# alipay/PainlessInferenceAcceleration

Hardware: NVIDIA H100
Metric: accepted tokens/sec @ Llama-2-7B 64-draft/8-branch; mean accepted len/step (higher is better)
Workload: dtype bf16

## Files before the change

painlessinferenceacceleration_b200/csrc/fused_ops.cu:

```cuda
#include <cuda_bf16.h>

#include "common.cuh"

namespace pia {
namespace fused {

__device__ __forceinline__ float bf(float x) { return __bfloat162float(__float2bfloat16_rn(x)); }

union Pack8 { uint4 u; __nv_bfloat16 h[8]; };

__device__ __forceinline__ Pack8 load_x8(const __nv_bfloat16 *x, const float *parts, int n_parts, long long part_stride,
                                         long long off) {
  Pack8 a;
  if (parts == nullptr) { a.u = *reinterpret_cast<const uint4 *>(x + off); return a; }
  float acc[8] = {0.f, 0.f, 0.f, 0.f, 0.f, 0.f, 0.f, 0.f};
  for (int s = 0; s < n_parts; ++s) {
    const float4 lo = *reinterpret_cast<const float4 *>(parts + s * part_stride + off);
    const float4 hi = *reinterpret_cast<const float4 *>(parts + s * part_stride + off + 4);
    acc[0] += lo.x; acc[1] += lo.y; acc[2] += lo.z; acc[3] += lo.w;
    acc[4] += hi.x; acc[5] += hi.y; acc[6] += hi.z; acc[7] += hi.w;
  }
#pragma unroll
  for (int j = 0; j < 8; ++j) a.h[j] = __float2bfloat16_rn(acc[j]);
  return a;
// ... 41 lines not shown
#pragma unroll
  for (int i = 0; i < 16; ++i) tot += red[i];
  const float inv = rsqrtf(tot / (float)hidden + eps);
  const uint4 *wv = reinterpret_cast<const uint4 *>(w);
  uint4 *yv = reinterpret_cast<uint4 *>(y + row_off);
#pragma unroll
  for (int k = 0; k < kRmsVec; ++k) {
    const int v = tid + k * 512;
    if (v < nvec) {
      Pack8 ww; ww.u = wv[v];
      Pack8 o;
#pragma unroll
      for (int j = 0; j < 8; ++j) {
        const float xh = __bfloat162float(keep[k].h[j]) * inv;
        o.h[j] = __float2bfloat16_rn(__bfloat162float(ww.h[j]) * (kRoundTwice ? bf(xh) : xh));
      }
      yv[v] = o.u;
    }
  }
}

enum { ROPE_HALF = 0, ROPE_INTERLEAVED = 1, ROPE_HALF_F32 = 2, ROPE_NONE = 3 };

__device__ __forceinline__ int tree_pos(const unsigned long long *mask, int mask_words, int i, int P, int pad_len,
                                        int max_pos) {
  int depth = -1;
  for (int w = 0; w < mask_words; ++w) depth += __popcll(mask[(long long)i * mask_words + w]);
  int pos = (P > pad_len ? P - pad_len : 0) + depth;
  if (pos < 0) pos = 0;
  if (pos >= max_pos) pos = max_pos - 1;
  return pos;
}

template <int kLayout, bool kLogn = false>
__global__ void __launch_bounds__(256) k_rope_kv_append(const __nv_bfloat16 *qkv, const unsigned long long *mask,
                                                        int mask_words, pia_slots_t sl,
                                                        int hq, int hkv, int hd, const void *cos_t,
                                                        const void *sin_t, int max_pos, __nv_bfloat16 *q_out,
                                                        __nv_bfloat16 *kc, __nv_bfloat16 *vc, int max_seq,
                                                        int rotary_dim, const __nv_bfloat16 *q_scale, int hd_src,
                                                        float q_mul) {
  static_assert(!kLogn || kLayout == ROPE_HALF_F32, "log-n scaling is built on the fp32 layout only");
  pdl_launch_dependents();
  pdl_wait();
  const int i = blockIdx.x;
  const int slot = i / sl.rows_per_slot, node = i % sl.rows_per_slot;
  const int n = sl.d_n[slot], P = sl.d_prefix_len[slot];
  const int pad_len = sl.d_pad_len ? sl.d_pad_len[slot] : 0;
  if (node >= n) return;
  kc += (long long)slot * sl.kv_slot_stride;
  vc += (long long)slot * sl.kv_slot_stride;
  if constexpr (kLayout == ROPE_NONE) {
    const int cpr = hd >> 3, cache_row = P + node;
    const __nv_bfloat16 *src = qkv + (long long)i * (hq + 2 * hkv) * hd_src;
    for (int c = threadIdx.x; c < (hq + 2 * hkv) * cpr; c += blockDim.x) {
      const int head = c / cpr, d0 = (c % cpr) * 8;
      Pack8 a;
      a.u = d0 < hd_src ? *reinterpret_cast<const uint4 *>(src + head * hd_src + d0) : make_uint4(0, 0, 0, 0);
      if (head < hq) {
#pragma unroll
        for (int j = 0; j < 8; ++j) a.h[j] = __float2bfloat16_rn(__fmul_rn(__bfloat162float(a.h[j]), q_mul));
        *reinterpret_cast<uint4 *>(q_out + ((long long)i * hq + head) * hd + d0) = a.u;
      } else if (head < hq + hkv) {
        *reinterpret_cast<uint4 *>(kc + ((long long)(head - hq) * max_seq + cache_row) * hd + d0) = a.u;
      } else {
        *reinterpret_cast<uint4 *>(vc + ((long long)(head - hq - hkv) * max_seq + cache_row) * hd + d0) = a.u;
      }
    }
    return;
  }
  const int pos = tree_pos(mask, mask_words, i, P, pad_len, max_pos);
  const int half = hd >> 1, cpr = hd >> 3;
  const int row_elems = (hq + 2 * hkv) * hd;
  const __nv_bfloat16 *src = qkv + (long long)i * row_elems;
  const int cache_row = P + node;
  const int total = (hq + 2 * hkv) * cpr;
  for (int c = threadIdx.x; c < total; c += blockDim.x) {
    const int head = c / cpr, ch = c % cpr;
    const int d0 = ch * 8;
    Pack8 a; a.u = *reinterpret_cast<const uint4 *>(src + head * hd + d0);
    if (head < hq + hkv) {
      Pack8 o;
      const __nv_bfloat16 *cos_b = static_cast<const __nv_bfloat16 *>(cos_t);
      const __nv_bfloat16 *sin_b = static_cast<const __nv_bfloat16 *>(sin_t);
      if constexpr (kLayout == ROPE_INTERLEAVED) {
        o = a;
        if (d0 < rotary_dim) {
          const int rhalf = rotary_dim >> 1;
          union { uint2 u; __nv_bfloat16 h[4]; } cs, sn;
          cs.u = *reinterpret_cast<const uint2 *>(cos_b + (long long)pos * rhalf + (d0 >> 1));
          sn.u = *reinterpret_cast<const uint2 *>(sin_b + (long long)pos * rhalf + (d0 >> 1));
#pragma unroll
          for (int j = 0; j < 4; ++j) {
            const float x0 = __bfloat162float(a.h[2 * j]), x1 = __bfloat162float(a.h[2 * j + 1]);
            const float c = __bfloat162float(cs.h[j]), s = __bfloat162float(sn.h[j]);
            o.h[2 * j] = __float2bfloat16_rn(bf(x0 * c) + bf(-x1 * s));
            o.h[2 * j + 1] = __float2bfloat16_rn(bf(x1 * c) + bf(x0 * s));
          }
        }
      } else if constexpr (kLayout == ROPE_HALF_F32) {
        const int dp = d0 < half ? d0 + half : d0 - half;
        Pack8 b; b.u = *reinterpret_cast<const uint4 *>(src + head * hd + dp);
        const float *cf = static_cast<const float *>(cos_t) + (long long)pos * half + d0 % half;
        const float *sf = static_cast<const float *>(sin_t) + (long long)pos * half + d0 % half;
        float c[8], s[8];
        *reinterpret_cast<float4 *>(c) = *reinterpret_cast<const float4 *>(cf);
        *reinterpret_cast<float4 *>(c + 4) = *reinterpret_cast<const float4 *>(cf + 4);
        *reinterpret_cast<float4 *>(s) = *reinterpret_cast<const float4 *>(sf);
        *reinterpret_cast<float4 *>(s + 4) = *reinterpret_cast<const float4 *>(sf + 4);
#pragma unroll
// ... 195 lines not shown
                              (const __nv_bfloat16 *)d_weight, eps, hidden, (__nv_bfloat16 *)d_residual_out,
                              (__nv_bfloat16 *)d_y));
  count_launch();
  return PIA_OK;
}

extern "C" int pia_rmsnorm(const void *d_x, const void *d_residual_in, const void *d_weight, float eps, int rounding,
                           int rows, int hidden, void *d_residual_out, void *d_y, void *stream) {
  PIA_REQUIRE(d_x, "bad rmsnorm arguments");
  return rmsnorm(d_x, nullptr, 0, 0ll, d_residual_in, d_weight, eps, rounding, rows, hidden, d_residual_out, d_y,
                 stream);
}

extern "C" int pia_rmsnorm_partials(const float *d_x_parts, int n_parts, int64_t part_stride, const void *d_residual_in,
                                    const void *d_weight, float eps, int rounding, int rows, int hidden,
                                    void *d_residual_out, void *d_y, void *stream) {
  PIA_REQUIRE(d_x_parts && n_parts >= 1, "bad rmsnorm arguments");
  return rmsnorm(nullptr, d_x_parts, n_parts, (long long)part_stride, d_residual_in, d_weight, eps, rounding, rows,
                 hidden, d_residual_out, d_y, stream);
}

template <int kLayout, bool kLogn = false>
static int rope_kv_append(const void *d_qkv, const uint64_t *d_mask, int mask_words, const pia_slots_t *slots,
                          int n_q_heads, int n_kv_heads, int head_dim, const void *d_cos, const void *d_sin, int max_pos,
                          void *d_q_out, void *d_k_cache_layer, void *d_v_cache_layer, int max_seq, int rotary_dim,
                          void *stream, const void *d_q_scale = nullptr, int hd_src = 0, float q_mul = 1.f) {
  PIA_REQUIRE(d_qkv && d_mask && slots && slots->d_n && slots->d_prefix_len && d_q_out && d_k_cache_layer &&
                  d_v_cache_layer && (kLayout == ROPE_NONE || (d_cos && d_sin)), "null argument");
  PIA_REQUIRE(slots->batch >= 1 && slots->rows_per_slot >= 1 && slots->kv_slot_stride >= 0, "bad slot table");
  PIA_REQUIRE(head_dim % 16 == 0 && mask_words >= 1 && mask_words <= 2, "bad rope arguments");
  PIA_REQUIRE(!kLogn || d_q_scale, "null argument");
  PIA_REQUIRE(kLayout != ROPE_NONE || (hd_src >= 8 && hd_src % 8 == 0 && hd_src <= head_dim),
              "bad source head width: a positive multiple of 8, at most head_dim");
  PIA_CUDA_CHECK(launch_kernel(k_rope_kv_append<kLayout, kLogn>, dim3(slots->batch * slots->rows_per_slot), dim3(256), 0,
                              (cudaStream_t)stream, (const __nv_bfloat16 *)d_qkv, (const unsigned long long *)d_mask,
                              mask_words, *slots, n_q_heads, n_kv_heads, head_dim, d_cos, d_sin, max_pos,
                              (__nv_bfloat16 *)d_q_out,
                              (__nv_bfloat16 *)d_k_cache_layer, (__nv_bfloat16 *)d_v_cache_layer, max_seq, rotary_dim,
                              (const __nv_bfloat16 *)d_q_scale, hd_src, q_mul));
  count_launch();
  return PIA_OK;
}

extern "C" int pia_kv_append_qscale(const void *d_qkv, const uint64_t *d_mask, int mask_words, const pia_slots_t *slots,
                                    int n_q_heads, int n_kv_heads, int src_head_dim, int head_dim, float q_mul,
                                    void *d_q_out, void *d_k_cache_layer, void *d_v_cache_layer, int max_seq,
                                    void *stream) {
  return rope_kv_append<ROPE_NONE>(d_qkv, d_mask, mask_words, slots, n_q_heads, n_kv_heads, head_dim, nullptr, nullptr,
                                   1, d_q_out, d_k_cache_layer, d_v_cache_layer, max_seq, head_dim, stream, nullptr,
                                   src_head_dim, q_mul);
}

extern "C" int pia_learned_pos_embed(const void *d_tok_table, const int32_t *d_ids, const void *d_pos_table,
                                     int offset, int max_pos, const uint64_t *d_mask, int mask_words,
                                     const pia_slots_t *slots, int hidden, void *d_out, void *stream) {
  PIA_REQUIRE(d_pos_table && d_mask && slots && slots->d_n && slots->d_prefix_len && d_out &&
                  (d_ids || !d_tok_table), "null argument");
  PIA_REQUIRE(slots->batch >= 1 && slots->rows_per_slot >= 1, "bad slot table");
  PIA_REQUIRE(hidden > 0 && hidden % 8 == 0 && offset >= 0 && max_pos >= 1 && mask_words >= 1 && mask_words <= 2,
              "bad position embedding arguments: hidden a positive multiple of 8, offset >= 0, max_pos >= 1");
  PIA_CUDA_CHECK(launch_kernel(k_learned_pos_embed, dim3(slots->batch * slots->rows_per_slot), dim3(256), 0,
                              (cudaStream_t)stream, (const __nv_bfloat16 *)d_tok_table, (const int *)d_ids,
                              (const __nv_bfloat16 *)d_pos_table, offset, max_pos, (const unsigned long long *)d_mask,
                              mask_words, *slots, hidden, (__nv_bfloat16 *)d_out));
  count_launch();
  return PIA_OK;
}
// ... 209 lines not shown
```

painlessinferenceacceleration_b200/csrc/tree_attn.cu:

```cuda
#include <cuda.h>
#include <cuda_bf16.h>

#include <stdlib.h>

#include <new>

#include "common.cuh"

namespace pia {
namespace attn {

constexpr int BN = 128;
constexpr int NSTAGE = 2;
constexpr int NTHREADS = 288;
constexpr int PRODUCER_WARP = 8;
constexpr int SUB = 128 * 128;
constexpr int MAX_SPLIT = 8;
constexpr int ALIBI_SLOPE = 64;
constexpr int ALIBI_DEPTH = 128;
constexpr float LOG2E = 1.4426950408889634f;

template <int HD>
struct Smem {
  static constexpr int TILE_BYTES = HD / 64 * SUB;
  static constexpr int Q = 0, K = TILE_BYTES, V = K + NSTAGE * TILE_BYTES;
  static constexpr int BAR = V + NSTAGE * TILE_BYTES;
  static constexpr int MRG_ACC = 0;
  static constexpr int MRG_ML = 7 * TILE_BYTES / 2;
  static constexpr int DED_ACC = BAR + 256, DED_ACC_BYTES = (64 + MAX_SPLIT) * HD * 4,
                       DED_ML = DED_ACC + DED_ACC_BYTES;
  static constexpr int TOTAL = DED_ML + 1024 + 1024;
  static_assert(MRG_ACC + HD / 4 * (128 + MAX_SPLIT) * 16 <= MRG_ML, "aliased partial rows overlap the (m, l) pairs");
  static_assert(MRG_ML + (128 + MAX_SPLIT) * 8 <= BAR, "aliased merge area reaches the barriers");
  static_assert(3 * NSTAGE * 8 <= ALIBI_SLOPE && ALIBI_SLOPE + 8 <= ALIBI_DEPTH && BAR + ALIBI_DEPTH + 128 <= DED_ACC,
                "ALiBi slopes / depths overlap");
};

__device__ __forceinline__ uint32_t smem_u32(const void *p) { return (uint32_t)__cvta_generic_to_shared(p); }
__device__ __forceinline__ void mbar_init(uint32_t bar, int count) {
  asm volatile("mbarrier.init.shared::cta.b64 [%0], %1;" ::"r"(bar), "r"(count));
}
__device__ __forceinline__ void mbar_arrive(uint32_t bar) {
  asm volatile("mbarrier.arrive.shared::cta.b64 _, [%0];" ::"r"(bar) : "memory");
}
__device__ __forceinline__ void mbar_expect_tx(uint32_t bar, uint32_t bytes) {
  asm volatile("mbarrier.arrive.expect_tx.shared::cta.b64 _, [%0], %1;" ::"r"(bar), "r"(bytes) : "memory");
}
__device__ __forceinline__ void mbar_wait(uint32_t bar, uint32_t parity) {
  uint32_t done;
  do {
    asm volatile(
        "{\n\t.reg .pred p;\n\t"
        "mbarrier.try_wait.parity.shared::cta.b64 p, [%1], %2;\n\t"
        "selp.u32 %0, 1, 0, p;\n\t}"
        : "=r"(done)
        : "r"(bar), "r"(parity)
        : "memory");
  } while (!done);
}
__device__ __forceinline__ void tma_load_3d(uint32_t dst, const CUtensorMap *map, uint32_t bar, int c0, int c1, int c2) {
  asm volatile(
      "cp.async.bulk.tensor.3d.shared::cluster.global.mbarrier::complete_tx::bytes [%0], [%1, {%3, %4, %5}], [%2];"
      ::"r"(dst), "l"(map), "r"(bar), "r"(c0), "r"(c1), "r"(c2)
      : "memory");
}
__device__ __forceinline__ void wgmma_fence() { asm volatile("wgmma.fence.sync.aligned;" ::: "memory"); }
__device__ __forceinline__ void wgmma_commit() { asm volatile("wgmma.commit_group.sync.aligned;" ::: "memory"); }
__device__ __forceinline__ void wgmma_wait_all() { asm volatile("wgmma.wait_group.sync.aligned 0;" ::: "memory"); }
// ... 20 lines not shown
      "{\n\t"
      "wgmma.mma_async.sync.aligned.m64n128k16.f32.bf16.bf16 "
      "{%0, %1, %2, %3, %4, %5, %6, %7, %8, %9, %10, %11, %12, %13, %14, %15, %16, %17, %18, %19, %20, %21, %22, %23, %24, %25, %26, %27, %28, %29, %30, %31, %32, %33, %34, %35, %36, %37, %38, %39, %40, %41, %42, %43, %44, %45, %46, %47, %48, %49, %50, %51, %52, %53, %54, %55, %56, %57, %58, %59, %60, %61, %62, %63}, {%64, %65, %66, %67}, %68, 1, 1, 1, 1;\n\t}"
      : "+f"(d[0]), "+f"(d[1]), "+f"(d[2]), "+f"(d[3]), "+f"(d[4]), "+f"(d[5]), "+f"(d[6]), "+f"(d[7]), "+f"(d[8]), "+f"(d[9]), "+f"(d[10]), "+f"(d[11]), "+f"(d[12]), "+f"(d[13]), "+f"(d[14]), "+f"(d[15]), "+f"(d[16]), "+f"(d[17]), "+f"(d[18]), "+f"(d[19]), "+f"(d[20]), "+f"(d[21]), "+f"(d[22]), "+f"(d[23]), "+f"(d[24]), "+f"(d[25]), "+f"(d[26]), "+f"(d[27]), "+f"(d[28]), "+f"(d[29]), "+f"(d[30]), "+f"(d[31]), "+f"(d[32]), "+f"(d[33]), "+f"(d[34]), "+f"(d[35]), "+f"(d[36]), "+f"(d[37]), "+f"(d[38]), "+f"(d[39]), "+f"(d[40]), "+f"(d[41]), "+f"(d[42]), "+f"(d[43]), "+f"(d[44]), "+f"(d[45]), "+f"(d[46]), "+f"(d[47]), "+f"(d[48]), "+f"(d[49]), "+f"(d[50]), "+f"(d[51]), "+f"(d[52]), "+f"(d[53]), "+f"(d[54]), "+f"(d[55]), "+f"(d[56]), "+f"(d[57]), "+f"(d[58]), "+f"(d[59]), "+f"(d[60]), "+f"(d[61]), "+f"(d[62]), "+f"(d[63])
      : "r"(a[0]), "r"(a[1]), "r"(a[2]), "r"(a[3]), "l"(desc_b)
      : "memory");
}
__device__ __forceinline__ void wgmma_pv(float (&d)[32], const uint32_t *a, uint64_t desc_b) {
  asm volatile(
      "{\n\t"
      "wgmma.mma_async.sync.aligned.m64n64k16.f32.bf16.bf16 "
      "{%0, %1, %2, %3, %4, %5, %6, %7, %8, %9, %10, %11, %12, %13, %14, %15, %16, %17, %18, %19, %20, %21, %22, %23, %24, %25, %26, %27, %28, %29, %30, %31}, {%32, %33, %34, %35}, %36, 1, 1, 1, 1;\n\t}"
      : "+f"(d[0]), "+f"(d[1]), "+f"(d[2]), "+f"(d[3]), "+f"(d[4]), "+f"(d[5]), "+f"(d[6]), "+f"(d[7]), "+f"(d[8]), "+f"(d[9]), "+f"(d[10]), "+f"(d[11]), "+f"(d[12]), "+f"(d[13]), "+f"(d[14]), "+f"(d[15]), "+f"(d[16]), "+f"(d[17]), "+f"(d[18]), "+f"(d[19]), "+f"(d[20]), "+f"(d[21]), "+f"(d[22]), "+f"(d[23]), "+f"(d[24]), "+f"(d[25]), "+f"(d[26]), "+f"(d[27]), "+f"(d[28]), "+f"(d[29]), "+f"(d[30]), "+f"(d[31])
      : "r"(a[0]), "r"(a[1]), "r"(a[2]), "r"(a[3]), "l"(desc_b)
      : "memory");
}
__device__ __forceinline__ float ex2(float x) {
  float y;
  asm("ex2.approx.ftz.f32 %0, %1;" : "=f"(y) : "f"(x));
  return y;
}
__device__ __forceinline__ void cluster_sync_all() {
  asm volatile("barrier.cluster.arrive.release.aligned;\n\tbarrier.cluster.wait.acquire.aligned;" ::: "memory");
}
__device__ __forceinline__ void cluster_arrive() { asm volatile("barrier.cluster.arrive.release.aligned;" ::: "memory"); }
__device__ __forceinline__ void cluster_wait() { asm volatile("barrier.cluster.wait.acquire.aligned;" ::: "memory"); }
__device__ __forceinline__ uint32_t map_to_cta(uint32_t local_smem_addr, uint32_t cta_rank) {
  uint32_t r;
  asm volatile("mapa.shared::cluster.u32 %0, %1, %2;" : "=r"(r) : "r"(local_smem_addr), "r"(cta_rank));
  return r;
}
__device__ __forceinline__ void st_cluster_f2(uint32_t addr, float a, float b) {
  asm volatile("st.shared::cluster.v2.f32 [%0], {%1, %2};" ::"r"(addr), "f"(a), "f"(b) : "memory");
}
__device__ __forceinline__ void fence_async_smem() { asm volatile("fence.proxy.async.shared::cta;" ::: "memory"); }

__device__ __forceinline__ uint64_t make_desc(uint32_t saddr, uint32_t lbo_bytes, uint32_t sbo_bytes) {
  uint64_t d = 0;
  d |= (uint64_t)((saddr >> 4) & 0x3FFF);
  d |= (uint64_t)((lbo_bytes >> 4) & 0x3FFF) << 16;
  d |= (uint64_t)((sbo_bytes >> 4) & 0x3FFF) << 32;
  d |= (uint64_t)1 << 62;
  return d;
}

union Pack8 { uint4 u; __nv_bfloat16 h[8]; };
__device__ __forceinline__ float bfr(float x) { return __bfloat162float(__float2bfloat16_rn(x)); }
__device__ __forceinline__ uint4 rope8(uint4 xa, uint4 xb, uint4 cs, uint4 sn, bool lower) {
  Pack8 a, b, c, s, o;
  a.u = xa; b.u = xb; c.u = cs; s.u = sn;
#pragma unroll
  for (int j = 0; j < 8; ++j) {
    const float x = __bfloat162float(a.h[j]);
    const float r = lower ? -__bfloat162float(b.h[j]) : __bfloat162float(b.h[j]);
    o.h[j] = __float2bfloat16_rn(bfr(x * __bfloat162float(c.h[j])) + bfr(r * __bfloat162float(s.h[j])));
  }
  return o.u;
}

struct Params {
  const __nv_bfloat16 *q;
  const unsigned long long *mask;
  pia_slots_t sl;
  int slot_planes;
  int plane0;
  int layer, n_q_heads, n_kv_heads, np, mask_words, heads_per_cta, max_seq, n_split, tiles_per_cta;
  int ctas_per_kv;
  float scale_log2;
  int fused;
  const __nv_bfloat16 *qkv;
  const __nv_bfloat16 *cos_t, *sin_t;
  int max_pos;
  __nv_bfloat16 *kc_layer, *vc_layer;
  __nv_bfloat16 *out;
  unsigned long long *dbg;
  const float *slopes;
};

__device__ __forceinline__ unsigned long long gtime() {
  unsigned long long t;
  asm volatile("mov.u64 %0, %%globaltimer;" : "=l"(t));
  return t;
}
struct HeadGroup { int hkv, j, hq0, heads; };
__device__ __forceinline__ HeadGroup head_group(const Params &p, int group) {
  const int G = p.n_q_heads / p.n_kv_heads;
  HeadGroup g;
  g.hkv = group / p.ctas_per_kv;
  g.j = group - g.hkv * p.ctas_per_kv;
  g.hq0 = g.hkv * G + g.j * p.heads_per_cta;
  g.heads = min(p.heads_per_cta, G - g.j * p.heads_per_cta);
  return g;
}

#define DBG(ev) do { if (p.dbg) p.dbg[((size_t)blockIdx.y * gridDim.x + blockIdx.x) * 16 + (ev)] = gtime(); } while (0)

template <int HD, bool kAlibi>
__global__ void __launch_bounds__(NTHREADS, 1)
k_tree_attn(const __grid_constant__ CUtensorMap map_k, const __grid_constant__ CUtensorMap map_v, Params p) {
  constexpr int TILE_BYTES = Smem<HD>::TILE_BYTES, SMEM_Q = Smem<HD>::Q, SMEM_K = Smem<HD>::K, SMEM_V = Smem<HD>::V;
  constexpr int SMEM_BAR = Smem<HD>::BAR, MRG_ACC = Smem<HD>::MRG_ACC, MRG_ML = Smem<HD>::MRG_ML;
  constexpr int MRG_DED_ACC = Smem<HD>::DED_ACC, MRG_DED_ACC_BYTES = Smem<HD>::DED_ACC_BYTES, MRG_DED_ML = Smem<HD>::DED_ML;
  constexpr int CH = HD / 16, HALF_SUB = HD == 128 ? SUB : 0, HALF_CH = HD == 128 ? 0 : CH;
  extern __shared__ uint8_t smem_raw[];
  const uint32_t base = (smem_u32(smem_raw) + 1023u) & ~1023u;
  uint8_t *sm = smem_raw + (base - smem_u32(smem_raw));
  const int tid = threadIdx.x, warp = tid >> 5, lane = tid & 31;

  const uint32_t bar0 = base + SMEM_BAR;
  const uint32_t bar_kv_full = bar0, bar_kv_empty = bar0 + 8 * NSTAGE, bar_v_full = bar0 + 16 * NSTAGE;

  pdl_launch_dependents();
  if (tid == 0) {
    asm volatile("prefetch.tensormap [%0];" ::"l"(reinterpret_cast<unsigned long long>(&map_k)) : "memory");
    asm volatile("prefetch.tensormap [%0];" ::"l"(reinterpret_cast<unsigned long long>(&map_v)) : "memory");
  }
  const int split = blockIdx.x, group = blockIdx.y;
  const int slot = blockIdx.z;
  const int n = p.sl.d_n[slot], P = p.sl.d_prefix_len[slot];
  const int pad_len = p.sl.d_pad_len ? p.sl.d_pad_len[slot] : 0;
  if (n <= 0) return;
  const long long row0 = (long long)slot * p.sl.rows_per_slot;
  const int L = P + n;
  const HeadGroup hg = head_group(p, group);
  const int hkv = hg.hkv, hq0 = hg.hq0, heads_here = hg.heads;
  const bool fused = !kAlibi && p.fused != 0;
  const int Tp = (P + BN - 1) / BN;
  const int tiles_total = fused ? Tp + 1 : (L + BN - 1) / BN;
  const int rows_used = heads_here * p.np;
  const int n_wg = rows_used / 64;
  const bool ded = (rows_used + MAX_SPLIT) * HD * 4 <= MRG_DED_ACC_BYTES;
  int ns = (tiles_total + p.tiles_per_cta - 1) / p.tiles_per_cta;
  if (ns > p.n_split) ns = p.n_split;
  if (ns < 1) ns = 1;
  if (split >= ns) {
    if (ns > 1) { cluster_sync_all(); cluster_sync_all(); }
    return;
  }
  const int tps = (tiles_total + ns - 1) / ns;
  const int t0 = split * tps;
  int t1 = t0 + tps;
  if (t1 > tiles_total) t1 = tiles_total;
  const int ntile = t1 - t0;
  const bool has_draft = fused && ntile > 0 && t1 == tiles_total;
  auto tile_of = [&](int i) -> int { return has_draft ? (i == 0 ? Tp : t0 + i - 1) : t0 + i; };
  if (ns > 1 && ded) cluster_arrive();
  auto barrier_a = [&]() { if (ded) cluster_wait(); else cluster_sync_all(); };
  const int mrg_acc = ded ? MRG_DED_ACC : MRG_ACC, mrg_ml = ded ? MRG_DED_ML : MRG_ML;
  const int mrg_stride = ded ? 64 + MAX_SPLIT : 128 + MAX_SPLIT;
  if (tid == 0) DBG(0);

  if (tid == 0) {
    for (int s = 0; s < NSTAGE; ++s) {
      mbar_init(bar_kv_full + 8 * s, 1); mbar_init(bar_v_full + 8 * s, 1);
      mbar_init(bar_kv_empty + 8 * s, 4 * n_wg);
    }
    asm volatile("fence.mbarrier_init.release.cluster;" ::: "memory");
  }
  __syncwarp();
  __syncthreads();
  if (tid == 0) DBG(1);

  if (warp == PRODUCER_WARP) {
    if (lane == 0 && ntile > 0) {
      const int plane = p.plane0 + slot * p.slot_planes + p.layer * p.n_kv_heads + hkv;
      int p_safe = P;
      if (p.slot_planes == 0) for (int b2 = 0; b2 < p.sl.batch; ++b2) p_safe = min(p_safe, p.sl.d_prefix_len[b2]);
      bool waited = false;
      for (int i = 0; i < ntile; ++i) {
        const int s = i % NSTAGE, ph = (i / NSTAGE) & 1;
        if (has_draft && i == 0) {
          mbar_arrive(bar_kv_full);
          mbar_arrive(bar_v_full);
          continue;
        }
        const int key0 = tile_of(i) * BN;
        if (!fused && !waited && key0 + BN > p_safe) { pdl_wait(); waited = true; }
        mbar_wait(bar_kv_empty + 8 * s, ph ^ 1);
        const uint32_t kd = base + SMEM_K + s * TILE_BYTES, vd = base + SMEM_V + s * TILE_BYTES;
        mbar_expect_tx(bar_kv_full + 8 * s, TILE_BYTES);
#pragma unroll
        for (int b = 0; b < HD / 64; ++b) tma_load_3d(kd + b * SUB, &map_k, bar_kv_full + 8 * s, 64 * b, key0, plane);
        mbar_expect_tx(bar_v_full + 8 * s, TILE_BYTES);
#pragma unroll
        for (int b = 0; b < HD / 64; ++b) tma_load_3d(vd + b * SUB, &map_v, bar_v_full + 8 * s, 64 * b, key0, plane);
        if (i == 0) DBG(2);
      }
    }
    __syncwarp();
    if (ns > 1) { barrier_a(); cluster_sync_all(); }
  } else {
    pdl_wait();
    {
      const int srow = tid & 127, half = tid >> 7;
      const int hs = srow / p.np, node = srow % p.np;
      if (srow < rows_used) {
        if (!fused) {
          uint4 qv[CH];
          const bool have = hs < heads_here && node < n;
          const uint4 *src = reinterpret_cast<const uint4 *>(p.q + ((row0 + node) * p.n_q_heads + hq0 + hs) * HD) + half * CH;
#pragma unroll
          for (int ch = 0; ch < CH; ++ch) qv[ch] = have ? src[ch] : make_uint4(0, 0, 0, 0);
#pragma unroll
          for (int ch = 0; ch < CH; ++ch)
            *reinterpret_cast<uint4 *>(sm + SMEM_Q + half * HALF_SUB + srow * 128 + (((half * HALF_CH + ch) ^ (srow & 7)) << 4)) = qv[ch];
        } else {
          unsigned long long mr0 = 0ull, mr1 = 0ull;
          if (node < n) {
            mr0 = p.mask[(row0 + node) * p.mask_words];
            if (p.mask_words > 1) mr1 = p.mask[(row0 + node) * p.mask_words + 1];
          }
          int pos = (P > pad_len ? P - pad_len : 0) + __popcll(mr0) + __popcll(mr1) - 1;
          pos = pos < 0 ? 0 : (pos >= p.max_pos ? p.max_pos - 1 : pos);
          const uint4 *cs = reinterpret_cast<const uint4 *>(p.cos_t + (long long)pos * (HD / 2));
          const uint4 *sn = reinterpret_cast<const uint4 *>(p.sin_t + (long long)pos * (HD / 2));
          const long long row_elems = (long long)(p.n_q_heads + 2 * p.n_kv_heads) * HD;
          const __nv_bfloat16 *xr = p.qkv + (row0 + node) * row_elems;
          const bool have = hs < heads_here && node < n;
          {
            const uint4 *qa = reinterpret_cast<const uint4 *>(xr + (long long)(hq0 + hs) * HD) + half * CH;
            const uint4 *qb = reinterpret_cast<const uint4 *>(xr + (long long)(hq0 + hs) * HD) + (half ^ 1) * CH;
#pragma unroll
            for (int b4 = 0; b4 < CH / 4; ++b4) {
// ... 233 lines not shown
        wgmma_fence();
#pragma unroll
        for (int j = 0; j < BN / 16; ++j) {
          wgmma_pv(o, pa + 4 * j, make_desc(va + j * 2048, SUB, 1024));
        }
        wgmma_commit();
        wgmma_wait_all();
        fence_regs(o);
        fence_regs(pa);
        __syncwarp();
        if (lane == 0) mbar_arrive(bar_kv_empty + 8 * s);
      }
      if (tid == 0) DBG(8);
      const HeadGroup hl = head_group(p, group);
#pragma unroll
      for (int h = 0; h < 2; ++h) {
        l_run[h] += __shfl_xor_sync(FULL, l_run[h], 1);
        l_run[h] += __shfl_xor_sync(FULL, l_run[h], 2);
      }
      if (tid == 0) DBG(9);
      if (ns == 1) {
#pragma unroll
        for (int h = 0; h < 2; ++h) {
          if (live[h]) {
            const float inv = l_run[h] > 0.f ? 1.f / l_run[h] : 0.f;
            uint32_t *dst = reinterpret_cast<uint32_t *>(p.out + ((row0 + node[h]) * p.n_q_heads + hl.hq0 + hs[h]) * HD);
#pragma unroll
            for (int nb = 0; nb < HD / 8; ++nb) {
              __nv_bfloat162 b = __floats2bfloat162_rn(o[4 * nb + 2 * h] * inv, o[4 * nb + 2 * h + 1] * inv);
              dst[4 * nb + (lane & 3)] = *reinterpret_cast<uint32_t *>(&b);
            }
          }
        }
      } else {
        barrier_a();
        if (tid == 0) DBG(14);
        const int RS = (hl.heads * p.np + ns - 1) / ns;
#pragma unroll
        for (int h = 0; h < 2; ++h) {
          if (live[h]) {
            const int owner = rw[h] / RS, rl = rw[h] % RS;
            const uint32_t dst = map_to_cta(base + mrg_acc + (uint32_t)((((lane & 3) >> 1) * mrg_stride + split * RS + rl) * 16 + (lane & 1) * 8), owner);
#pragma unroll
            for (int nb = 0; nb < HD / 8; ++nb)
              st_cluster_f2(dst + (uint32_t)(2 * nb * mrg_stride) * 16, o[4 * nb + 2 * h], o[4 * nb + 2 * h + 1]);
            if ((lane & 3) == 0) st_cluster_f2(map_to_cta(base + mrg_ml + (uint32_t)(split * RS + rl) * 8, owner), m_run[h], l_run[h]);
          }
        }
        __syncwarp();
        if (tid == 0) DBG(15);
        cluster_sync_all();
      }
      if (tid == 0) DBG(10);
    } else {
      if (ns > 1) { barrier_a(); cluster_sync_all(); }
    }
  }
  if (ns > 1) {
    const HeadGroup hl = head_group(p, group);
    const int rows_late = hl.heads * p.np;
    const int RS = (rows_late + ns - 1) / ns;
    const float4 *macc = reinterpret_cast<const float4 *>(sm + mrg_acc);
    const float2 *mml = reinterpret_cast<const float2 *>(sm + mrg_ml);
    const int items = RS * (HD / 4);
    const bool pow2 = (RS & (RS - 1)) == 0 && (p.np & (p.np - 1)) == 0;
    const int rs_sh = 31 - __clz(RS), np_sh = 31 - __clz(p.np);
    for (int it = tid; it < items; it += NTHREADS) {
      const int rl = pow2 ? (it & (RS - 1)) : it % RS, c4 = pow2 ? (it >> rs_sh) : it / RS;
      const int r = split * RS + rl;
      if (r >= rows_late) continue;
      const int rh = pow2 ? (r >> np_sh) : r / p.np, rn = pow2 ? (r & (p.np - 1)) : r % p.np;
      if (rn >= n) continue;
      float2 ml[MAX_SPLIT];
      float4 a4[MAX_SPLIT];
#pragma unroll
      for (int i = 0; i < MAX_SPLIT; ++i) {
        if (i < ns) { ml[i] = mml[i * RS + rl]; a4[i] = macc[c4 * mrg_stride + i * RS + rl]; }
        else { ml[i] = make_float2(-INFINITY, 0.f); a4[i] = make_float4(0.f, 0.f, 0.f, 0.f); }
      }
      float M = -INFINITY;
#pragma unroll
      for (int i = 0; i < MAX_SPLIT; ++i) M = fmaxf(M, ml[i].x);
      float den = 0.f;
      float4 o4 = make_float4(0.f, 0.f, 0.f, 0.f);
#pragma unroll
      for (int i = 0; i < MAX_SPLIT; ++i) {
        const float w = ml[i].x == -INFINITY ? 0.f : ex2(ml[i].x - M);
        den += ml[i].y * w;
        o4.x += a4[i].x * w; o4.y += a4[i].y * w; o4.z += a4[i].z * w; o4.w += a4[i].w * w;
      }
      const float inv = den > 0.f ? 1.f / den : 0.f;
      __nv_bfloat162 b0 = __floats2bfloat162_rn(o4.x * inv, o4.y * inv), b1 = __floats2bfloat162_rn(o4.z * inv, o4.w * inv);
      reinterpret_cast<uint2 *>(p.out + ((row0 + rn) * p.n_q_heads + hl.hq0 + rh) * HD)[c4] =
          make_uint2(*reinterpret_cast<uint32_t *>(&b0), *reinterpret_cast<uint32_t *>(&b1));
    }
  }
  if (tid == 0) DBG(12);
}

}
}

using namespace pia;
using namespace pia::attn;

struct pia_attn_plan {
  pia_attn_config_t cfg;
  CUtensorMap map_k, map_v;
  int heads_per_cta, ctas_per_kv, n_groups, n_split, mask_words, tiles_per_cta;
  unsigned long long *dbg;
  __nv_bfloat16 *k_base, *v_base;
};

typedef CUresult (*EncodeTiledFn)(CUtensorMap *, CUtensorMapDataType, cuuint32_t, void *, const cuuint64_t *,
                                  const cuuint64_t *, const cuuint32_t *, const cuuint32_t *, CUtensorMapInterleave,
                                  CUtensorMapSwizzle, CUtensorMapL2promotion, CUtensorMapFloatOOBfill);

static int encode_kv_map(CUtensorMap *m, void *base, const pia_attn_config_t &c) {
  static EncodeTiledFn fn = nullptr;
  if (!fn) {
    cudaDriverEntryPointQueryResult qres;
    void *ptr = nullptr;
    PIA_CUDA_CHECK(cudaGetDriverEntryPoint("cuTensorMapEncodeTiled", &ptr, cudaEnableDefault, &qres));
    PIA_REQUIRE(ptr && qres == cudaDriverEntryPointSuccess, "cuTensorMapEncodeTiled not available in this driver");
    fn = (EncodeTiledFn)ptr;
  }
  cuuint64_t dims[3] = {(cuuint64_t)c.head_dim, (cuuint64_t)c.max_seq,
                        (cuuint64_t)(c.n_slots > 0 ? c.n_slots : 1) * c.n_layers * c.n_kv_heads};
  cuuint64_t strides[2] = {(cuuint64_t)c.head_dim * 2, (cuuint64_t)c.max_seq * c.head_dim * 2};
  cuuint32_t box[3] = {64, (cuuint32_t)BN, 1};
  cuuint32_t estr[3] = {1, 1, 1};
  CUresult r = fn(m, CU_TENSOR_MAP_DATA_TYPE_BFLOAT16, 3, base, dims, strides, box, estr, CU_TENSOR_MAP_INTERLEAVE_NONE,
                  CU_TENSOR_MAP_SWIZZLE_128B, CU_TENSOR_MAP_L2_PROMOTION_L2_256B, CU_TENSOR_MAP_FLOAT_OOB_FILL_NONE);
  if (r != CUDA_SUCCESS) { set_error("cuTensorMapEncodeTiled failed with CUresult %d", (int)r); return PIA_ERR_CUDA; }
  return PIA_OK;
}

extern "C" int pia_attn_plan_create(const pia_attn_config_t *cfg, void *d_k_cache, void *d_v_cache,
                                    pia_attn_plan_t **out) {
  PIA_REQUIRE(cfg && d_k_cache && d_v_cache && out, "null argument");
  if (cfg->head_dim != 64 && cfg->head_dim != 128) {
    set_error("head_dim %d: k_tree_attn is built for 64 and 128", cfg->head_dim);
    return PIA_ERR_UNSUPPORTED;
  }
// ... 2 lines not shown
  PIA_REQUIRE(cfg->max_seq > 0 && cfg->n_layers > 0, "bad cache shape");
  PIA_REQUIRE((reinterpret_cast<uintptr_t>(d_k_cache) & 15) == 0 && (reinterpret_cast<uintptr_t>(d_v_cache) & 15) == 0, "cache must be 16-byte aligned");
  pia_attn_plan *p = new (std::nothrow) pia_attn_plan();
  PIA_REQUIRE(p, "out of host memory");
  p->cfg = *cfg;
  const int G = cfg->n_q_heads / cfg->n_kv_heads;
  p->heads_per_cta = cfg->max_nodes == 64 ? 2 : 1;
  p->ctas_per_kv = (G + p->heads_per_cta - 1) / p->heads_per_cta;
  p->n_groups = cfg->n_kv_heads * p->ctas_per_kv;
  p->mask_words = cfg->max_nodes / 64;
  int n_sm = 132, dev = 0;
  cudaGetDevice(&dev);
  cudaDeviceGetAttribute(&n_sm, cudaDevAttrMultiProcessorCount, dev);
  const int max_tiles = (cfg->max_seq + BN - 1) / BN;
  int ns = cfg->kv_split_max > 0 ? cfg->kv_split_max : n_sm / p->n_groups;
  if (ns > max_tiles) ns = max_tiles;
  if (ns < 1) ns = 1;
  if (ns > MAX_SPLIT) ns = MAX_SPLIT;
  p->n_split = ns;
  p->tiles_per_cta = 1;
  if (const char *e = getenv("PIA_ATTN_TILES_PER_CTA")) { int v = atoi(e); if (v >= 1 && v <= 64) p->tiles_per_cta = v; }
  int rc = encode_kv_map(&p->map_k, d_k_cache, *cfg);
  if (rc == PIA_OK) rc = encode_kv_map(&p->map_v, d_v_cache, *cfg);
  if (rc == PIA_OK) {
    cudaError_t e = cfg->head_dim == 64
                        ? cudaFuncSetAttribute(k_tree_attn<64, false>, cudaFuncAttributeMaxDynamicSharedMemorySize, Smem<64>::TOTAL)
                        : cudaFuncSetAttribute(k_tree_attn<128, false>, cudaFuncAttributeMaxDynamicSharedMemorySize, Smem<128>::TOTAL);
    if (e == cudaSuccess && cfg->head_dim == 128)
      e = cudaFuncSetAttribute(k_tree_attn<128, true>, cudaFuncAttributeMaxDynamicSharedMemorySize, Smem<128>::TOTAL);
    if (e != cudaSuccess) { set_error("cudaFuncSetAttribute: %s", cudaGetErrorString(e)); rc = PIA_ERR_CUDA; }
  }
  p->dbg = nullptr;
  p->k_base = (__nv_bfloat16 *)d_k_cache; p->v_base = (__nv_bfloat16 *)d_v_cache;
  if (rc != PIA_OK) { delete p; return rc; }
  *out = p;
  return PIA_OK;
}

extern "C" int pia_attn_plan_set_debug(pia_attn_plan_t *p, void *d_timestamps) {
  PIA_REQUIRE(p, "null plan");
  p->dbg = (unsigned long long *)d_timestamps;
  return PIA_OK;
}
extern "C" int pia_attn_plan_grid(const pia_attn_plan_t *p, int *n_split, int *n_groups) {
  PIA_REQUIRE(p && n_split && n_groups, "null argument");
  *n_split = p->n_split; *n_groups = p->n_groups;
  return PIA_OK;
}

extern "C" int pia_attn_plan_destroy(pia_attn_plan_t *p) {
  if (p) delete p;
  return PIA_OK;
}

static int attn_launch(pia_attn_plan_t *p, int layer, const void *d_q, const void *d_qkv, const void *d_cos,
                       const void *d_sin, int max_pos, const uint64_t *d_mask, const pia_slots_t *slots, float scale_mul,
                       void *d_out, void *stream, const float *d_slopes = nullptr) {
  const bool fused = d_qkv != nullptr;
  PIA_REQUIRE(p && (d_q || d_qkv) && d_mask && slots && slots->d_n && slots->d_prefix_len && d_out, "null argument");
  if (d_slopes && p->cfg.head_dim != 128) {
    set_error("head_dim %d: the ALiBi tree attention is built for head_dim 128 only", p->cfg.head_dim);
    return PIA_ERR_UNSUPPORTED;
  }
  PIA_REQUIRE(layer >= 0 && layer < p->cfg.n_layers, "layer %d outside [0,%d)", layer, p->cfg.n_layers);
  PIA_REQUIRE(slots->batch >= 1 && slots->batch <= 65535 && slots->rows_per_slot >= 1 &&
                  slots->rows_per_slot <= p->cfg.max_nodes, "bad slot table");
  const long long cache_elems = (long long)p->cfg.n_layers * p->cfg.n_kv_heads * p->cfg.max_seq * p->cfg.head_dim;
  const int plan_slots = p->cfg.n_slots > 0 ? p->cfg.n_slots : 1;
  PIA_REQUIRE(slots->kv_first_slot >= 0 && slots->kv_first_slot < plan_slots, "kv_first_slot outside the plan's caches");
  PIA_REQUIRE(slots->kv_slot_stride == 0 || (slots->kv_slot_stride == cache_elems &&
                                              slots->kv_first_slot + slots->batch <= plan_slots),
              "kv_slot_stride must be 0 or one whole cache, and the plan must span `batch` caches");
  PIA_REQUIRE(!fused || slots->batch == 1 || slots->kv_slot_stride != 0,
              "the fused RoPE / KV-append attention needs one cache per slot");
  PIA_REQUIRE(!fused || (d_cos && d_sin && max_pos > 0), "fused mode needs the RoPE tables");
  Params a;
  a.q = (const __nv_bfloat16 *)d_q;
  a.mask = (const unsigned long long *)d_mask;
  a.sl = *slots;
  a.slot_planes = slots->kv_slot_stride ? p->cfg.n_layers * p->cfg.n_kv_heads : 0;
  a.plane0 = slots->kv_first_slot * p->cfg.n_layers * p->cfg.n_kv_heads;
  a.layer = layer; a.n_q_heads = p->cfg.n_q_heads; a.n_kv_heads = p->cfg.n_kv_heads; a.np = p->cfg.max_nodes;
  a.mask_words = p->mask_words; a.max_seq = p->cfg.max_seq;
  a.heads_per_cta = p->heads_per_cta; a.ctas_per_kv = p->ctas_per_kv;
  int ns = p->n_split / slots->batch;
  if (ns < 1) ns = 1;
  a.n_split = ns; a.tiles_per_cta = p->tiles_per_cta;
  a.out = (__nv_bfloat16 *)d_out; a.dbg = p->dbg;
  a.fused = fused ? 1 : 0;
  a.qkv = (const __nv_bfloat16 *)d_qkv; a.cos_t = (const __nv_bfloat16 *)d_cos; a.sin_t = (const __nv_bfloat16 *)d_sin;
  a.max_pos = max_pos;
  const long long layer_off = ((long long)slots->kv_first_slot * p->cfg.n_layers + layer) * p->cfg.n_kv_heads *
                              (long long)p->cfg.max_seq * p->cfg.head_dim;
  a.kc_layer = p->k_base + layer_off; a.vc_layer = p->v_base + layer_off;
  a.scale_log2 = scale_mul * 1.4426950408889634f / sqrtf((float)p->cfg.head_dim);
  a.slopes = d_slopes;
  cudaStream_t s = (cudaStream_t)stream;
  const dim3 grid(ns, p->n_groups, slots->batch);
  if (d_slopes)
    PIA_CUDA_CHECK(launch_kernel_cluster(k_tree_attn<128, true>, grid, dim3(NTHREADS), Smem<128>::TOTAL, s,
                                         (unsigned)ns, p->map_k, p->map_v, a));
  else if (p->cfg.head_dim == 64)
    PIA_CUDA_CHECK(launch_kernel_cluster(k_tree_attn<64, false>, grid, dim3(NTHREADS), Smem<64>::TOTAL, s, (unsigned)ns,
                                         p->map_k, p->map_v, a));
  else
    PIA_CUDA_CHECK(launch_kernel_cluster(k_tree_attn<128, false>, grid, dim3(NTHREADS), Smem<128>::TOTAL, s, (unsigned)ns,
                                         p->map_k, p->map_v, a));
  count_launch();
  return PIA_OK;
}

extern "C" int pia_tree_attn_fwd(pia_attn_plan_t *p, int layer, const void *d_q, const uint64_t *d_mask,
                                 const pia_slots_t *slots, float scale_mul, void *d_out, void *stream) {
  PIA_REQUIRE(d_q, "null q");
  return attn_launch(p, layer, d_q, nullptr, nullptr, nullptr, 0, d_mask, slots, scale_mul, d_out, stream);
}

extern "C" int pia_tree_attn_fused_fwd(pia_attn_plan_t *p, int layer, const void *d_qkv, const void *d_cos,
                                       const void *d_sin, int max_pos, const uint64_t *d_mask, const pia_slots_t *slots,
                                       float scale_mul, void *d_out, void *stream) {
  PIA_REQUIRE(d_qkv, "null qkv");
  return attn_launch(p, layer, nullptr, d_qkv, d_cos, d_sin, max_pos, d_mask, slots, scale_mul, d_out, stream);
}

extern "C" int pia_tree_attn_alibi_fwd(pia_attn_plan_t *p, int layer, const void *d_q, const uint64_t *d_mask,
                                       const pia_slots_t *slots, float scale_mul, const float *d_slopes, void *d_out,
                                       void *stream) {
  PIA_REQUIRE(d_q && d_slopes, "null q / slopes");
  return attn_launch(p, layer, d_q, nullptr, nullptr, nullptr, 0, d_mask, slots, scale_mul, d_out, stream, d_slopes);
}
```

Baseline: 582.9.

## Merge split-KV attention via global workspace and split RoPE append across CTAs

When there is one head group and 64 nodes, split-KV tree attention drops the cluster launch. Each split writes its partial accumulators and max/sum to a global workspace, and the last CTA to arrive, found with an atomic counter, does the combine. For the cluster path, the second cluster-wide sync is replaced by remote mbarrier arrivals with a cluster fence. The RoPE/KV-append kernel now runs 128-thread blocks on a 2D grid so each row's chunks spread over several CTAs. This trades extra global traffic and an atomic for fewer cluster barriers and freer scheduling, and it adds workspace sizing limits on batch.

```diff
diff --git a/painlessinferenceacceleration_b200/csrc/fused_ops.cu b/painlessinferenceacceleration_b200/csrc/fused_ops.cu
--- a/painlessinferenceacceleration_b200/csrc/fused_ops.cu
+++ b/painlessinferenceacceleration_b200/csrc/fused_ops.cu
@@ -97,8 +97,10 @@
   return pos;
 }
 
+constexpr int kRopeThreads = 128;
+
 template <int kLayout, bool kLogn = false>
-__global__ void __launch_bounds__(256) k_rope_kv_append(const __nv_bfloat16 *qkv, const unsigned long long *mask,
+__global__ void __launch_bounds__(kRopeThreads) k_rope_kv_append(const __nv_bfloat16 *qkv, const unsigned long long *mask,
                                                         int mask_words, pia_slots_t sl,
                                                         int hq, int hkv, int hd, const void *cos_t,
                                                         const void *sin_t, int max_pos, __nv_bfloat16 *q_out,
@@ -118,7 +120,7 @@
   if constexpr (kLayout == ROPE_NONE) {
     const int cpr = hd >> 3, cache_row = P + node;
     const __nv_bfloat16 *src = qkv + (long long)i * (hq + 2 * hkv) * hd_src;
-    for (int c = threadIdx.x; c < (hq + 2 * hkv) * cpr; c += blockDim.x) {
+    for (int c = blockIdx.y * blockDim.x + threadIdx.x; c < (hq + 2 * hkv) * cpr; c += gridDim.y * blockDim.x) {
       const int head = c / cpr, d0 = (c % cpr) * 8;
       Pack8 a;
       a.u = d0 < hd_src ? *reinterpret_cast<const uint4 *>(src + head * hd_src + d0) : make_uint4(0, 0, 0, 0);
@@ -140,7 +142,7 @@
   const __nv_bfloat16 *src = qkv + (long long)i * row_elems;
   const int cache_row = P + node;
   const int total = (hq + 2 * hkv) * cpr;
-  for (int c = threadIdx.x; c < total; c += blockDim.x) {
+  for (int c = blockIdx.y * blockDim.x + threadIdx.x; c < total; c += gridDim.y * blockDim.x) {
     const int head = c / cpr, ch = c % cpr;
     const int d0 = ch * 8;
     Pack8 a; a.u = *reinterpret_cast<const uint4 *>(src + head * hd + d0);
@@ -402,7 +404,10 @@
   PIA_REQUIRE(!kLogn || d_q_scale, "null argument");
   PIA_REQUIRE(kLayout != ROPE_NONE || (hd_src >= 8 && hd_src % 8 == 0 && hd_src <= head_dim),
               "bad source head width: a positive multiple of 8, at most head_dim");
-  PIA_CUDA_CHECK(launch_kernel(k_rope_kv_append<kLayout, kLogn>, dim3(slots->batch * slots->rows_per_slot), dim3(256), 0,
+  const int chunks = (n_q_heads + 2 * n_kv_heads) * (head_dim / 8);
+  PIA_CUDA_CHECK(launch_kernel(k_rope_kv_append<kLayout, kLogn>,
+                              dim3(slots->batch * slots->rows_per_slot, (chunks + kRopeThreads - 1) / kRopeThreads),
+                              dim3(kRopeThreads), 0,
                               (cudaStream_t)stream, (const __nv_bfloat16 *)d_qkv, (const unsigned long long *)d_mask,
                               mask_words, *slots, n_q_heads, n_kv_heads, head_dim, d_cos, d_sin, max_pos,
                               (__nv_bfloat16 *)d_q_out,
diff --git a/painlessinferenceacceleration_b200/csrc/tree_attn.cu b/painlessinferenceacceleration_b200/csrc/tree_attn.cu
--- a/painlessinferenceacceleration_b200/csrc/tree_attn.cu
+++ b/painlessinferenceacceleration_b200/csrc/tree_attn.cu
@@ -16,6 +16,8 @@
 constexpr int PRODUCER_WARP = 8;
 constexpr int SUB = 128 * 128;
 constexpr int MAX_SPLIT = 8;
+constexpr int WS_ROWS = 64;
+constexpr int WS_STRIDE = MAX_SPLIT * WS_ROWS;
 constexpr int ALIBI_SLOPE = 64;
 constexpr int ALIBI_DEPTH = 128;
 constexpr float LOG2E = 1.4426950408889634f;
@@ -34,6 +36,8 @@
   static_assert(MRG_ML + (128 + MAX_SPLIT) * 8 <= BAR, "aliased merge area reaches the barriers");
   static_assert(3 * NSTAGE * 8 <= ALIBI_SLOPE && ALIBI_SLOPE + 8 <= ALIBI_DEPTH && BAR + ALIBI_DEPTH + 128 <= DED_ACC,
                 "ALiBi slopes / depths overlap");
+  static constexpr int BAR_MRG = 3 * NSTAGE * 8;
+  static_assert(BAR_MRG + 8 <= ALIBI_SLOPE, "merge barrier overlaps the ALiBi slopes");
 };
 
 __device__ __forceinline__ uint32_t smem_u32(const void *p) { return (uint32_t)__cvta_generic_to_shared(p); }
@@ -120,6 +124,22 @@
 }
 __device__ __forceinline__ void st_cluster_f2(uint32_t addr, float a, float b) {
   asm volatile("st.shared::cluster.v2.f32 [%0], {%1, %2};" ::"r"(addr), "f"(a), "f"(b) : "memory");
+}
+__device__ __forceinline__ void fence_cluster() { asm volatile("fence.acq_rel.cluster;" ::: "memory"); }
+__device__ __forceinline__ void mbar_arrive_remote(uint32_t cluster_addr) {
+  asm volatile("mbarrier.arrive.release.cluster.shared::cluster.b64 _, [%0];" ::"r"(cluster_addr) : "memory");
+}
+__device__ __forceinline__ void mbar_wait_cluster(uint32_t bar, uint32_t parity) {
+  uint32_t done;
+  do {
+    asm volatile(
+        "{\n\t.reg .pred p;\n\t"
+        "mbarrier.try_wait.parity.acquire.cluster.shared::cta.b64 p, [%1], %2;\n\t"
+        "selp.u32 %0, 1, 0, p;\n\t}"
+        : "=r"(done)
+        : "r"(bar), "r"(parity)
+        : "memory");
+  } while (!done);
 }
 __device__ __forceinline__ void fence_async_smem() { asm volatile("fence.proxy.async.shared::cta;" ::: "memory"); }
 
@@ -163,7 +183,12 @@
   __nv_bfloat16 *out;
   unsigned long long *dbg;
   const float *slopes;
+  int gmerge;
+  float *ws;
+  int *ws_cnt;
 };
+template <int HD>
+constexpr int ws_group_floats() { return HD / 4 * WS_STRIDE * 4 + WS_STRIDE * 2; }
 
 __device__ __forceinline__ unsigned long long gtime() {
   unsigned long long t;
@@ -197,6 +222,7 @@
 
   const uint32_t bar0 = base + SMEM_BAR;
   const uint32_t bar_kv_full = bar0, bar_kv_empty = bar0 + 8 * NSTAGE, bar_v_full = bar0 + 16 * NSTAGE;
+  const uint32_t bar_mrg = base + SMEM_BAR + Smem<HD>::BAR_MRG;
 
   pdl_launch_dependents();
   if (tid == 0) {
@@ -221,8 +247,9 @@
   int ns = (tiles_total + p.tiles_per_cta - 1) / p.tiles_per_cta;
   if (ns > p.n_split) ns = p.n_split;
   if (ns < 1) ns = 1;
+  const bool gm = p.gmerge != 0;
   if (split >= ns) {
-    if (ns > 1) { cluster_sync_all(); cluster_sync_all(); }
+    if (ns > 1 && !gm) cluster_sync_all();
     return;
   }
   const int tps = (tiles_total + ns - 1) / ns;
@@ -232,7 +259,6 @@
   const int ntile = t1 - t0;
   const bool has_draft = fused && ntile > 0 && t1 == tiles_total;
   auto tile_of = [&](int i) -> int { return has_draft ? (i == 0 ? Tp : t0 + i - 1) : t0 + i; };
-  if (ns > 1 && ded) cluster_arrive();
   auto barrier_a = [&]() { if (ded) cluster_wait(); else cluster_sync_all(); };
   const int mrg_acc = ded ? MRG_DED_ACC : MRG_ACC, mrg_ml = ded ? MRG_DED_ML : MRG_ML;
   const int mrg_stride = ded ? 64 + MAX_SPLIT : 128 + MAX_SPLIT;
@@ -243,10 +269,12 @@
       mbar_init(bar_kv_full + 8 * s, 1); mbar_init(bar_v_full + 8 * s, 1);
       mbar_init(bar_kv_empty + 8 * s, 4 * n_wg);
     }
+    if (ns > 1 && !gm) mbar_init(bar_mrg, ns * 4 * n_wg);
     asm volatile("fence.mbarrier_init.release.cluster;" ::: "memory");
   }
   __syncwarp();
   __syncthreads();
+  if (ns > 1 && ded && !gm) cluster_arrive();
   if (tid == 0) DBG(1);
 
   if (warp == PRODUCER_WARP) {
@@ -276,7 +304,7 @@
       }
     }
     __syncwarp();
-    if (ns > 1) { barrier_a(); cluster_sync_all(); }
+    if (ns > 1 && !gm) barrier_a();
   } else {
     pdl_wait();
     {
@@ -576,6 +604,20 @@
             }
           }
         }
+      } else if (p.gmerge) {
+        float *wa = p.ws + ((size_t)blockIdx.z * gridDim.y + blockIdx.y) * ws_group_floats<HD>();
+        float *wm = wa + HD / 4 * WS_STRIDE * 4;
+#pragma unroll
+        for (int h = 0; h < 2; ++h) {
+          if (live[h]) {
+            float *dst = wa + (size_t)(((lane & 3) >> 1) * WS_STRIDE + split * WS_ROWS + rw[h]) * 4 + (lane & 1) * 2;
+#pragma unroll
+            for (int nb = 0; nb < HD / 8; ++nb)
+              *reinterpret_cast<float2 *>(dst + (size_t)(2 * nb * WS_STRIDE) * 4) = make_float2(o[4 * nb + 2 * h], o[4 * nb + 2 * h + 1]);
+            if ((lane & 3) == 0) *reinterpret_cast<float2 *>(wm + (size_t)(split * WS_ROWS + rw[h]) * 2) = make_float2(m_run[h], l_run[h]);
+          }
+        }
+        if (tid == 0) DBG(15);
       } else {
         barrier_a();
         if (tid == 0) DBG(14);
@@ -591,52 +633,78 @@
             if ((lane & 3) == 0) st_cluster_f2(map_to_cta(base + mrg_ml + (uint32_t)(split * RS + rl) * 8, owner), m_run[h], l_run[h]);
           }
         }
+        fence_cluster();
         __syncwarp();
+        if (lane < ns) mbar_arrive_remote(map_to_cta(bar_mrg, lane));
         if (tid == 0) DBG(15);
-        cluster_sync_all();
       }
       if (tid == 0) DBG(10);
     } else {
-      if (ns > 1) { barrier_a(); cluster_sync_all(); }
+      if (ns > 1 && !gm) barrier_a();
     }
   }
   if (ns > 1) {
     const HeadGroup hl = head_group(p, group);
     const int rows_late = hl.heads * p.np;
-    const int RS = (rows_late + ns - 1) / ns;
-    const float4 *macc = reinterpret_cast<const float4 *>(sm + mrg_acc);
-    const float2 *mml = reinterpret_cast<const float2 *>(sm + mrg_ml);
-    const int items = RS * (HD / 4);
-    const bool pow2 = (RS & (RS - 1)) == 0 && (p.np & (p.np - 1)) == 0;
-    const int rs_sh = 31 - __clz(RS), np_sh = 31 - __clz(p.np);
-    for (int it = tid; it < items; it += NTHREADS) {
-      const int rl = pow2 ? (it & (RS - 1)) : it % RS, c4 = pow2 ? (it >> rs_sh) : it / RS;
-      const int r = split * RS + rl;
-      if (r >= rows_late) continue;
-      const int rh = pow2 ? (r >> np_sh) : r / p.np, rn = pow2 ? (r & (p.np - 1)) : r % p.np;
-      if (rn >= n) continue;
-      float2 ml[MAX_SPLIT];
-      float4 a4[MAX_SPLIT];
-#pragma unroll
-      for (int i = 0; i < MAX_SPLIT; ++i) {
-        if (i < ns) { ml[i] = mml[i * RS + rl]; a4[i] = macc[c4 * mrg_stride + i * RS + rl]; }
-        else { ml[i] = make_float2(-INFINITY, 0.f); a4[i] = make_float4(0.f, 0.f, 0.f, 0.f); }
+    auto combine = [&](int RS, int own, auto ld_ml, auto ld_acc) {
+      const int items = RS * (HD / 4);
+      const bool pow2 = (RS & (RS - 1)) == 0 && (p.np & (p.np - 1)) == 0;
+      const int rs_sh = 31 - __clz(RS), np_sh = 31 - __clz(p.np);
+      for (int it = tid; it < items; it += NTHREADS) {
+        const int rl = pow2 ? (it & (RS - 1)) : it % RS, c4 = pow2 ? (it >> rs_sh) : it / RS;
+        const int r = own * RS + rl;
+        if (r >= rows_late) continue;
+        const int rh = pow2 ? (r >> np_sh) : r / p.np, rn = pow2 ? (r & (p.np - 1)) : r % p.np;
+        if (rn >= n) continue;
+        float2 ml[MAX_SPLIT];
+        float4 a4[MAX_SPLIT];
+#pragma unroll
+        for (int i = 0; i < MAX_SPLIT; ++i) {
+          if (i < ns) { ml[i] = ld_ml(i * RS + rl); a4[i] = ld_acc(c4, i * RS + rl); }
+          else { ml[i] = make_float2(-INFINITY, 0.f); a4[i] = make_float4(0.f, 0.f, 0.f, 0.f); }
+        }
+        float M = -INFINITY;
+#pragma unroll
+        for (int i = 0; i < MAX_SPLIT; ++i) M = fmaxf(M, ml[i].x);
+        float den = 0.f;
+        float4 o4 = make_float4(0.f, 0.f, 0.f, 0.f);
+#pragma unroll
+        for (int i = 0; i < MAX_SPLIT; ++i) {
+          const float w = ml[i].x == -INFINITY ? 0.f : ex2(ml[i].x - M);
+          den += ml[i].y * w;
+          o4.x += a4[i].x * w; o4.y += a4[i].y * w; o4.z += a4[i].z * w; o4.w += a4[i].w * w;
+        }
+        const float inv = den > 0.f ? 1.f / den : 0.f;
+        __nv_bfloat162 b0 = __floats2bfloat162_rn(o4.x * inv, o4.y * inv), b1 = __floats2bfloat162_rn(o4.z * inv, o4.w * inv);
+        reinterpret_cast<uint2 *>(p.out + ((row0 + rn) * p.n_q_heads + hl.hq0 + rh) * HD)[c4] =
+            make_uint2(*reinterpret_cast<uint32_t *>(&b0), *reinterpret_cast<uint32_t *>(&b1));
       }
-      float M = -INFINITY;
-#pragma unroll
-      for (int i = 0; i < MAX_SPLIT; ++i) M = fmaxf(M, ml[i].x);
-      float den = 0.f;
-      float4 o4 = make_float4(0.f, 0.f, 0.f, 0.f);
-#pragma unroll
-      for (int i = 0; i < MAX_SPLIT; ++i) {
-        const float w = ml[i].x == -INFINITY ? 0.f : ex2(ml[i].x - M);
-        den += ml[i].y * w;
-        o4.x += a4[i].x * w; o4.y += a4[i].y * w; o4.z += a4[i].z * w; o4.w += a4[i].w * w;
+    };
+    if (p.gmerge) {
+      __threadfence();
+      __syncthreads();
+      int *last = reinterpret_cast<int *>(sm + SMEM_BAR + Smem<HD>::BAR_MRG);
+      if (tid == 0) {
+        int *cnt = p.ws_cnt + (size_t)blockIdx.z * gridDim.y + blockIdx.y;
+        *last = atomicAdd(cnt, 1) == ns - 1;
+        if (*last) *cnt = 0;
       }
-      const float inv = den > 0.f ? 1.f / den : 0.f;
-      __nv_bfloat162 b0 = __floats2bfloat162_rn(o4.x * inv, o4.y * inv), b1 = __floats2bfloat162_rn(o4.z * inv, o4.w * inv);
-      reinterpret_cast<uint2 *>(p.out + ((row0 + rn) * p.n_q_heads + hl.hq0 + rh) * HD)[c4] =
-          make_uint2(*reinterpret_cast<uint32_t *>(&b0), *reinterpret_cast<uint32_t *>(&b1));
+      __syncthreads();
+      if (!*last) {
+        if (tid == 0) DBG(12);
+        return;
+      }
+      __threadfence();
+      const float *wa = p.ws + ((size_t)blockIdx.z * gridDim.y + blockIdx.y) * ws_group_floats<HD>();
+      const float2 *wm = reinterpret_cast<const float2 *>(wa + HD / 4 * WS_STRIDE * 4);
+      const float4 *wacc = reinterpret_cast<const float4 *>(wa);
+      combine(WS_ROWS, 0, [&](int k) { return __ldcg(wm + k); }, [&](int c4, int k) { return __ldcg(wacc + c4 * WS_STRIDE + k); });
+    } else {
+      mbar_wait_cluster(bar_mrg, 0);
+      const float4 *macc = reinterpret_cast<const float4 *>(sm + mrg_acc);
+      const float2 *mml = reinterpret_cast<const float2 *>(sm + mrg_ml);
+      combine((rows_late + ns - 1) / ns, split, [&](int k) { return mml[k]; },
+              [&](int c4, int k) { return macc[c4 * mrg_stride + k]; });
     }
   }
   if (tid == 0) DBG(12);
@@ -654,6 +722,9 @@
   int heads_per_cta, ctas_per_kv, n_groups, n_split, mask_words, tiles_per_cta;
   unsigned long long *dbg;
   __nv_bfloat16 *k_base, *v_base;
+  int gmerge, ws_slots;
+  float *ws;
+  int *ws_cnt;
 };
 
 typedef CUresult (*EncodeTiledFn)(CUtensorMap *, CUtensorMapDataType, cuuint32_t, void *, const cuuint64_t *,
@@ -722,7 +793,18 @@
   }
   p->dbg = nullptr;
   p->k_base = (__nv_bfloat16 *)d_k_cache; p->v_base = (__nv_bfloat16 *)d_v_cache;
-  if (rc != PIA_OK) { delete p; return rc; }
+  p->gmerge = G == 1 && cfg->max_nodes == 64 && ns > 1;
+  p->ws = nullptr; p->ws_cnt = nullptr; p->ws_slots = 0;
+  if (rc == PIA_OK && p->gmerge) {
+    p->ws_slots = ns / 2 > 1 ? ns / 2 : 1;
+    const size_t groups = (size_t)p->ws_slots * p->n_groups;
+    const size_t floats = cfg->head_dim == 64 ? ws_group_floats<64>() : ws_group_floats<128>();
+    cudaError_t e = cudaMalloc(&p->ws, groups * floats * sizeof(float));
+    if (e == cudaSuccess) e = cudaMalloc(&p->ws_cnt, groups * sizeof(int));
+    if (e == cudaSuccess) e = cudaMemset(p->ws_cnt, 0, groups * sizeof(int));
+    if (e != cudaSuccess) { set_error("attention merge workspace: %s", cudaGetErrorString(e)); rc = PIA_ERR_CUDA; }
+  }
+  if (rc != PIA_OK) { cudaFree(p->ws); cudaFree(p->ws_cnt); delete p; return rc; }
   *out = p;
   return PIA_OK;
 }
@@ -739,7 +821,7 @@
 }
 
 extern "C" int pia_attn_plan_destroy(pia_attn_plan_t *p) {
-  if (p) delete p;
+  if (p) { cudaFree(p->ws); cudaFree(p->ws_cnt); delete p; }
   return PIA_OK;
 }
 
@@ -785,16 +867,20 @@
   a.kc_layer = p->k_base + layer_off; a.vc_layer = p->v_base + layer_off;
   a.scale_log2 = scale_mul * 1.4426950408889634f / sqrtf((float)p->cfg.head_dim);
   a.slopes = d_slopes;
+  a.gmerge = p->gmerge && ns > 1;
+  PIA_REQUIRE(!a.gmerge || slots->batch <= p->ws_slots, "merge workspace sized for %d slots", p->ws_slots);
+  a.ws = p->ws; a.ws_cnt = p->ws_cnt;
+  const unsigned cluster = a.gmerge ? 1u : (unsigned)ns;
   cudaStream_t s = (cudaStream_t)stream;
   const dim3 grid(ns, p->n_groups, slots->batch);
   if (d_slopes)
     PIA_CUDA_CHECK(launch_kernel_cluster(k_tree_attn<128, true>, grid, dim3(NTHREADS), Smem<128>::TOTAL, s,
-                                         (unsigned)ns, p->map_k, p->map_v, a));
+                                         cluster, p->map_k, p->map_v, a));
   else if (p->cfg.head_dim == 64)
-    PIA_CUDA_CHECK(launch_kernel_cluster(k_tree_attn<64, false>, grid, dim3(NTHREADS), Smem<64>::TOTAL, s, (unsigned)ns,
+    PIA_CUDA_CHECK(launch_kernel_cluster(k_tree_attn<64, false>, grid, dim3(NTHREADS), Smem<64>::TOTAL, s, cluster,
                                          p->map_k, p->map_v, a));
   else
-    PIA_CUDA_CHECK(launch_kernel_cluster(k_tree_attn<128, false>, grid, dim3(NTHREADS), Smem<128>::TOTAL, s, (unsigned)ns,
+    PIA_CUDA_CHECK(launch_kernel_cluster(k_tree_attn<128, false>, grid, dim3(NTHREADS), Smem<128>::TOTAL, s, cluster,
                                          p->map_k, p->map_v, a));
   count_launch();
   return PIA_OK;
```

New measurement: 595.6 (median of 6 runs). 1.02x the previous value.
